# microsoft/ISLE

Measured on AMD Instinct MI355X. Metric: docs/sec end-to-end ISLETrain (SVD+k-means), k=1000; top-k σ rel-err, higher is better.
Workload: dtype f32

## Files before the change

include/isle_hip.h:

```cpp
#ifndef ISLE_HIP_H
#define ISLE_HIP_H

#include <stddef.h>
#include <stdint.h>

#ifdef __cplusplus
extern "C" {
#endif

typedef struct isle_ctx isle_ctx;

enum {
  ISLE_OK = 0,
  ISLE_E_ARG = -1,
  ISLE_E_HIP = -2,
  ISLE_E_NOCONV = -3,
  ISLE_E_NUMERIC = -4,
  ISLE_E_COMM = -5
};

isle_ctx* isle_hip_create(int device_id);
void isle_hip_destroy(isle_ctx* ctx);
const char* isle_hip_last_error(isle_ctx* ctx);

// ... 39 lines not shown
                   uint64_t* original_cols, float* zetas);
int isle_hip_shape(isle_ctx* ctx, uint64_t* vocab_size, uint64_t* num_docs, uint64_t* nnz,
                   uint64_t* doc_offset, uint64_t* docs_global);

int isle_hip_frobenius(isle_ctx* ctx, float* out);

int isle_hip_gram_apply(isle_ctx* ctx, const float* X_colmajor, int b, float* Z_colmajor);

int isle_hip_operator_form(isle_ctx* ctx, int* form);

int isle_hip_switch_info(int index, const char** name, const char** kind, const char** what);

int isle_hip_block_ks(isle_ctx* ctx, int nev, int ncv, int maxit, int blk, float tol, uint64_t seed,
                      float* evals, int* nconv, int* restarts, int* napplies);

int isle_hip_block_ks_dense(isle_ctx* ctx, const float* A_colmajor, uint64_t n, int nev, int ncv, int maxit, int blk,
                            float tol, uint64_t seed, const float* start_block, float* evals, float* U_colmajor,
                            int* nconv, int* nconv_ref_rule, int* restarts, int* napplies);

int isle_hip_get_U(isle_ctx* ctx, float* U_colmajor);
int isle_hip_set_U(isle_ctx* ctx, const float* U_colmajor, int k);

int isle_hip_eig_sym(isle_ctx* ctx, const float* S_colmajor, int n, float* evals_desc, float* vecs_colmajor);

int isle_hip_kmeanspp_projected(isle_ctx* ctx, int k, const uint64_t* inject_seeds, uint64_t rng_seed,
                                uint64_t* seeds_out, float* C_lowd, float* residual, int* rounds);

int isle_hip_host_rand(uint64_t seed, int n, uint32_t* out);

int isle_hip_get_min_dist(isle_ctx* ctx, float* min_dist);

int isle_hip_lloyds_projected(isle_ctx* ctx, int k, float* C_lowd, int max_reps, int* iters_run,
                              uint32_t* assign_out);

int isle_hip_lift_centers(isle_ctx* ctx, const float* in, int ld_in, int ncols, float* centers);

int isle_hip_lloyds_sparse(isle_ctx* ctx, int k, const float* centers_in, float* centers_out,
                           uint32_t* assign, int max_reps, int* iters_run);

int isle_hip_catchwords(isle_ctx* ctx, int num_topics, const uint32_t* assign, uint64_t r, double rho,
                        float* thresholds, int32_t* catch_topic, uint64_t* num_catchwords);

int isle_hip_topic_model(isle_ctx* ctx, int num_topics, uint64_t rank_threshold, float* model,
                         float* model_threshold, int32_t* top1, int32_t* top2, uint64_t* doc_topic_sums);
int isle_hip_get_doc_topic_sums(isle_ctx* ctx, int64_t* doc_offsets, uint32_t* topic, float* val);

int isle_hip_edge_topics(isle_ctx* ctx, const int64_t* pairs, int n, float primary_ratio, float* edge);

#define ISLE_EDGE_TABLE_MAX_TOPICS 8192
int isle_hip_select_edge_pairs(isle_ctx* ctx, const int32_t* top1, const int32_t* top2, uint64_t n_docs, int num_topics,
                               int64_t max_edge_topics, uint64_t min_docs, int64_t* pairs, uint64_t cap, uint64_t* n_selected,
                               uint64_t* n_candidates, uint64_t* threshold );

int isle_hip_topic_coherence(isle_ctx* ctx, int num_topics, int M, const uint32_t* top_words, double eps, double* coherence,
                             uint64_t* doc_freq, uint64_t* co_doc_freq);

int isle_hip_avg_topic_model(isle_ctx* ctx, int num_topics, float* model);

#define ISLE_MODEL_CATCH 0
#define ISLE_MODEL_AVG 1
#define ISLE_MODEL_HOST 2
#define ISLE_MODEL_LOADED 3

int isle_hip_model_top_words(isle_ctx* ctx, int which, const float* model_host, uint64_t vocab, int ncols, int n, uint32_t* ids, float* weights);

int isle_hip_edge_top_words(isle_ctx* ctx, int which, const float* model_host, uint64_t vocab, int ncols, const int64_t* pairs, int n_edge,
// ... 79 lines not shown
```

isle_amd/_lib.py:

```python
import ctypes as C
import os

_HERE = os.path.dirname(os.path.abspath(__file__))
_LIB = None

_P, _I, _U64, _F = C.c_void_p, C.c_int, C.c_uint64, C.c_float
SYMBOLS = {
    "isle_hip_create": (_P, [_I]),
    "isle_hip_destroy": (None, [_P]),
    "isle_hip_last_error": (C.c_char_p, [_P]),
    "isle_hip_switch_info": (_I, [_I, _P, _P, _P]),
    "isle_hip_comm_unique_id": (_I, [_P]),
    "isle_hip_comm_init": (_I, [_P, _I, _I, _P]),
    "isle_hip_comm_init_host": (_I, [_P, _I, _I, _P, _P]),
    "isle_hip_plan_shards": (_I, [_U64, _P, _I, _P]),
    "isle_hip_upload_csc_u64": (_I, [_P, _U64, _U64, _U64, _P, _P, _P, _U64, _U64]),
    "isle_hip_upload_csc_u32": (_I, [_P, _U64, _U64, _U64, _P, _P, _P, _U64, _U64]),
    "isle_hip_upload_counts_u32": (_I, [_P, _U64, _U64, _U64, _P, _P, _P, _U64, _U64]),
    "isle_hip_ingest_tdf": (_I, [_P, _P, _U64, _U64, _U64, _U64, _P, _P]),
    "isle_hip_feed_begin": (_I, [_P, _U64, _U64, _U64]),
    "isle_hip_feed_entries": (_I, [_P, _U64, _P, _P, _P]),
    "isle_hip_feed_entries_pieces": (_I, [_P, _U64, _P, _P, _P, _U64]),
    "isle_hip_feed_finalize": (_I, [_P, _U64, _U64, _P, _P]),
    "isle_hip_tdf_begin": (_I, [_P, _U64, _U64, _U64, _U64]),
# ... 14 lines not shown
    "isle_hip_topic_coherence": (_I, [_P, _I, _I, _P, C.c_double, _P, _P, _P]),
    "isle_hip_avg_topic_model": (_I, [_P, _I, _P]),
    "isle_hip_model_top_words": (_I, [_P, _I, _P, _U64, _I, _I, _P, _P]),
    "isle_hip_topic_diversity": (_I, [_P, _I, _I, _P, _P]),
    "isle_hip_model_text": (_I, [_P, _I, _P, _U64, _I, _I, _P, _P, _P, _P]),
    "isle_hip_edge_topics_text": (_I, [_P, _P, _I, _F, _I, _P, _P, _P, _P]),
    "isle_hip_entry_text": (_I, [_F, _I, _P]),
    "isle_hip_load_model_text": (_I, [_P, _P, _U64, _U64, _I, _I, C.c_uint, _P]),
    "isle_hip_get_loaded_model": (_I, [_P, _P, _P, _P]),
    "isle_hip_parse_weight": (_I, [_P, _U64, _I, _P]),
    "isle_hip_log_combinatorial": (_I, [_P, _P, _P]),
    "isle_hip_distinct_top_five": (_I, [_P, _I, _P, _P, _P, _P, _P, _P]),
    "isle_hip_top_five_count_rule": (_I, [_P, _U64, C.c_int32, _P]),
    "isle_hip_frobenius": (_I, [_P, _P]),
    "isle_hip_gram_apply": (_I, [_P, _P, _I, _P]),
    "isle_hip_operator_form": (_I, [_P, _P]),
    "isle_hip_infer": (_I, [_P, C.c_uint64, _I, _P, C.c_uint64, C.c_uint64, _P, _P, _P, _I, C.c_float, C.c_float, _P, _P, _P, _P, _P]),
    "isle_hip_infer_resident": (_I, [_P, _I, _P, _U64, _I, _U64, _U64, _I, _F, _F, _U64, _P, _P, _P, _P, _P]),
    "isle_hip_get_infer_entries": (_I, [_P, _P, _P, _P]),
    "isle_hip_infer_text": (_I, [_P, _I, _U64, _U64, _U64, _P, _P, _P, _P]),
    "isle_hip_doc_line_text": (_I, [_U64, _U64, _F, _P]),
    "isle_hip_doc_report_text": (_I, [_P, _I, _U64, _U64, _P, _P, _P, _P]),
    "isle_hip_top_two_line_text": (_I, [_U64, _U64, _U64, _P]),
    "isle_hip_avg_doc_sz": (_I, [_P, _P]),
    "isle_hip_block_ks": (_I, [_P, _I, _I, _I, _I, _F, _U64, _P, _P, _P, _P]),
    "isle_hip_block_ks_dense": (_I, [_P, _P, _U64, _I, _I, _I, _I, _F, _U64, _P, _P, _P, _P, _P, _P, _P]),
    "isle_hip_get_U": (_I, [_P, _P]),
    "isle_hip_set_U": (_I, [_P, _P, _I]),
    "isle_hip_eig_sym": (_I, [_P, _P, _I, _P, _P]),
    "isle_hip_kmeanspp_projected": (_I, [_P, _I, _P, _U64, _P, _P, _P, _P]),
    "isle_hip_get_min_dist": (_I, [_P, _P]),
    "isle_hip_host_rand": (_I, [_U64, _I, _P]),
    "isle_hip_lloyds_projected": (_I, [_P, _I, _P, _I, _P, _P]),
    "isle_hip_lift_centers": (_I, [_P, _P, _I, _I, _P]),
    "isle_hip_lloyds_sparse": (_I, [_P, _I, _P, _P, _P, _I, _P]),
    "isle_hip_timing_enable": (_I, [_P, _I]),
    "isle_hip_timing_reset": (_I, [_P]),
    "isle_hip_timing_get": (_I, [_P, _P, _P]),
    "isle_hip_synchronize": (_I, [_P]),
}


class IsleHipError(RuntimeError):
    pass


def library_path():
    return os.environ.get("ISLE_HIP_LIB") or os.path.join(_HERE, "libisle_hip.so")


def load_library():
    global _LIB
    if _LIB is not None:
        return _LIB
    path = library_path()
    if not os.path.exists(path):
        raise IsleHipError(
            "%s not found — build it with `make -C isle_amd/csrc` (or __graft_entry__.build()). "
            "There is no CPU fallback for the ISLE hot path." % path)
    lib = C.CDLL(path)
    for name, (res, args) in SYMBOLS.items():
        fn = getattr(lib, name)
        fn.restype = res
        fn.argtypes = args
    _LIB = lib
    return lib
# ... 1 lines not shown
```

isle_amd/csrc/api_kmeans.cpp:

```cpp
#include <algorithm>
#include <chrono>
#include <cmath>
#include <cstdarg>
#include <cstdlib>
#include <cstring>
#include <numeric>

#include "api_internal.h"

#ifndef ISLE_PROJ_FULL_NUM
#define ISLE_PROJ_FULL_NUM 1
#define ISLE_PROJ_FULL_DEN 3
#endif
static void choose_movers(const std::vector<float>& delta, int k, int group, int G, YyMovers* mv, std::vector<float>* gmax_excl,
                          const std::vector<uint32_t>* slot_of_id = nullptr ) {
  mv->n = 0;
  if ((int)delta.size() != k || k <= 16) return;
  std::vector<int> ord(k);
  std::iota(ord.begin(), ord.end(), 0);
  std::partial_sort(ord.begin(), ord.begin() + 11, ord.end(), [&](int a, int b) { return delta[a] > delta[b] || (delta[a] == delta[b] && a < b); });
  const float ref = delta[ord[10]];
  for (int j = 0; j < 10; ++j)
    if (delta[ord[j]] > 2.0f * ref && delta[ord[j]] > 1e-4f) mv->id[mv->n++] = (uint32_t)ord[j];
  if (!mv->n) return;
// ... 302 lines not shown
  bool from_kmpp;
  bool pt_sorted;
  bool delta_sums;
  bool movers;
};
struct ProjScalars {
  float* delta;
  HamTop* top;
  float* tmove;
};
}

static ProjPlan proj_plan(isle_ctx* c, int k, const float* C_lowd) {
  ProjPlan p;
  p.hamerly = !c->knob_on(KN_NO_HAMERLY) && (c->Pt_ready || c->Pt2_ready);
  p.T = (k + 31) / 32;
  p.TL = (p.T + 3) & ~3;
  p.tiles = p.hamerly && k > 224 && p.T <= 32 && !c->knob_is(KN_PROJ_BOUNDS, "hamerly");
  p.from_kmpp = p.tiles && c->kmpp_track_k == k && c->kmpp_P_gen == c->P_gen && c->P_ready && !c->knob_zero(KN_KMPP_TRACK) &&
                c->kmpp_C_host.size() == (size_t)k * k && memcmp(c->kmpp_C_host.data(), C_lowd, (size_t)k * k * sizeof(float)) == 0;
  p.pt_sorted = !c->knob_zero(KN_PT_SORT);
  p.delta_sums = !c->knob_is(KN_PROJ_SUMS, "fresh") && c->D < (1ull << 31);
  p.movers = !c->knob_zero(KN_YY_MOVERS) && c->D > 0;
  return p;
}

static int proj_reserve(isle_ctx* c, const ProjPlan& p, int k, ProjScalars* sc) {
  const uint64_t D = c->D;
  const int ldk = c->ldk;
  if (p.hamerly) {
    HIPCHK(c, c->hub.reserve(D ? D : 1));
    HIPCHK(c, c->hlb.reserve(D ? D : 1));
    HIPCHK(c, c->active.reserve(D + 1));
    HIPCHK(c, c->Pa.reserve((size_t)(D ? D : 1) * ldk));
    HIPCHK(c, c->pna.reserve(D ? D : 1));
    HIPCHK(c, c->Cold.reserve((size_t)k * ldk + k + 8));
  }
  if (p.tiles) {
    HIPCHK(c, c->ptlb.reserve((size_t)(D ? D : 1) * p.TL));
    HIPCHK(c, c->pneed.reserve(D ? D : 1));
    HIPCHK(c, c->pcand.reserve(D + 1));
    HIPCHK(c, c->small.reserve(4096));
  }
  if (p.delta_sums) HIPCHK(c, c->proj_counted.reserve(D ? D : 1));
  if (c->multi()) HIPCHK(c, c->Csum_local.reserve((size_t)k * ldk));
  sc->delta = p.hamerly ? c->Cold.p + (size_t)k * ldk : nullptr;
  sc->top = p.hamerly ? reinterpret_cast<HamTop*>(c->Cold.p + (size_t)k * ldk + round4(k)) : nullptr;
  sc->tmove = p.tiles ? c->small.p : nullptr;
  return 0;
}

static int proj_assign_first(isle_ctx* c, const ProjPlan& p, int k) {
  const uint64_t D = c->D;
  const int ldk = c->ldk;
  if (p.from_kmpp) return k_kmpp_to_tiles(c, D, k, c->pnorm.p, c->cnorm.p, c->kmpp_best.p, c->assign.p, c->hub.p, p.TL);
  if (p.tiles)
    return k_proj_assign_tiles(c, c->P.p, c->pnorm.p, D, k, ldk, c->Cdev.p, c->cnorm.p, c->assign.p, c->hub.p, c->ptlb.p, p.TL, nullptr, 0, nullptr, nullptr,
                               nullptr);
  return k_proj_assign(c, c->P.p, c->pnorm.p, D, k, ldk, c->Cdev.p, c->cnorm.p, c->assign.p, p.hamerly ? c->hub.p : nullptr,
                       p.hamerly ? c->hlb.p : nullptr);
}

static int debug_tile_stats(isle_ctx* c, int it, uint32_t na, int T) {
  const uint64_t D = c->D;
  std::vector<uint32_t> act(na), need(D);
  if (na) HIPCHK(c, hipMemcpy(act.data(), c->active.p, na * sizeof(uint32_t), hipMemcpyDeviceToHost));
  if (D) HIPCHK(c, hipMemcpy(need.data(), c->pneed.p, D * sizeof(uint32_t), hipMemcpyDeviceToHost));
// ... 109 lines not shown
  HIPCHK(c, hipStreamSynchronize(c->stream));
  isle_host_mark("lloyds_projected: centres uploaded");
  ProjScalars sc;
  ISLECHK(proj_reserve(c, plan, k, &sc));
  c->kmpp_track_k = 0;
  if (c->knob_on(KN_DEBUG_HAMERLY)) fprintf(stderr, "[projected Lloyd] first assignment %s\n", plan.from_kmpp ? "taken from the k-means++ rounds" : "computed");
  StopRule stop(c, k);
  int it = 0;
  std::vector<float> pdelta_host;
  isle_host_mark("lloyds_projected: loop starts");
  for (; it < max_reps; ++it) {
    ISLECHK(k_rownorms(c, c->Cdev.p, k, k, ldk, c->cnorm.p));
    if (it == 0 || !plan.hamerly) ISLECHK(proj_assign_first(c, plan, k));
    else if (plan.tiles) ISLECHK(proj_reassign_tiles(c, plan, sc, k, it, pdelta_host));
    else ISLECHK(proj_reassign_hamerly(c, sc, k, it));
    ISLECHK(k_count_sizes(c, c->assign.p, D, k, c->counts.p));
    std::vector<long long> sizes;
    ISLECHK(proj_update_centres(c, plan, k, it, sizes));
    if (plan.hamerly && it + 1 < max_reps) ISLECHK(proj_movements(c, plan, sc, k, pdelta_host));
    bool conv = false;
    ISLECHK(stop.converged(sizes, c->assign.p, &conv));
    if (conv) {
      ++it;
      break;
    }
  }
  isle_host_mark("lloyds_projected: loop done");
  HIPCHK(c, hipMemcpyAsync(Ch, c->Cdev.p, ch_bytes, hipMemcpyDeviceToHost, c->stream));
  if (assign_out && D) HIPCHK(c, hipMemcpyAsync(assign_out, c->assign.p, D * sizeof(uint32_t), hipMemcpyDeviceToHost, c->stream));
  HIPCHK(c, hipStreamSynchronize(c->stream));
  centres_unpack(C_lowd, Ch, k, ldk);
  if (iters_run) *iters_run = it;
  isle_host_mark("lloyds_projected: exit");
  return 0;
}

static int install_centers(isle_ctx* c, int ncols) {
  const int ld = round4(ncols);
  HIPCHK(c, c->centers_rm.reserve((size_t)c->V * ld));
  HIPCHK(c, hipMemsetAsync(c->centers_rm.p, 0, (size_t)c->V * ld * sizeof(float), c->stream));
  ISLECHK(k_transpose(c, c->centers_cm.p, c->V, ncols, c->V, c->centers_rm.p, ld));
  c->centers_ready = true;
  c->centers_k = ncols;
  return 0;
}

extern "C" int isle_hip_lift_centers(isle_ctx* c, const float* in, int ld_in, int ncols, float* centers) {
  if (!c || !in || ncols < 1) return ISLE_E_ARG;
  ISLECHK(isle_enter(c));
  if (c->U_k == 0 || ld_in < c->U_k) return isle_fail(c, ISLE_E_ARG, "lift: need U and ld_in >= k");
  isle_host_mark("lift: entry");
  HIPCHK(c, c->Csum.reserve((size_t)ld_in * ncols));
  {
    const size_t in_bytes = (size_t)ld_in * ncols * sizeof(float);
    HIPCHK(c, c->pin_stage.reserve(in_bytes));
    memcpy(c->pin_stage.p, in, in_bytes);
    HIPCHK(c, hipMemcpyAsync(c->Csum.p, c->pin_stage.p, in_bytes, hipMemcpyHostToDevice, c->stream));
  }
  HIPCHK(c, c->centers_cm.reserve((size_t)c->V * ncols));
  ISLECHK(k_gemm_nn(c, c->Ucm.p, c->V, c->U_k, c->Csum.p, ld_in, ncols, c->centers_cm.p, ISLE_T_LIFT));
  ISLECHK(install_centers(c, ncols));
  HIPCHK(c, c->lift_C.reserve((size_t)ld_in * ncols));
  HIPCHK(c, hipMemcpyAsync(c->lift_C.p, c->Csum.p, (size_t)ld_in * ncols * sizeof(float), hipMemcpyDeviceToDevice, c->stream));
  c->lift_ld = ld_in;
  c->lift_k = ncols;
  c->lift_valid = true;
// ... 326 lines not shown
```

isle_amd/csrc/common.h:

```cpp
#pragma once
#include <hip/hip_runtime.h>
#include <rccl/rccl.h>

#include <atomic>
#include <cstdint>
#include <cstdio>
#include <functional>
#include <string>
#include <thread>
#include <vector>

#include "gl_plan.h"

struct IsleLaunchRefused {
  const char* file = nullptr;
  int line = 0;
  unsigned long long threads = 0;
};
inline IsleLaunchRefused& isle_launch_refused() {
  static thread_local IsleLaunchRefused r;
  return r;
}
inline bool isle_launch_fits(dim3 g, dim3 b, const char* file, int line) {
  const unsigned long long blocks = (unsigned long long)g.x * g.y * g.z, threads = blocks * ((unsigned long long)b.x * b.y * b.z);
// ... 557 lines not shown
int k_load_model_text(isle_ctx* c, const unsigned char* text_dev, uint64_t n, uint64_t V, uint32_t ncols, int format, unsigned base, float* model_dev,
                      uint64_t* nentries, uint64_t* err_key);

int k_coherence_counts(isle_ctx* c, const std::vector<uint32_t>& U, const std::vector<uint32_t>& part_off, const std::vector<uint32_t>& part_hi,
                       std::vector<uint32_t>& counts, int* passes);

int k_avg_model(isle_ctx* c, uint32_t k);
int k_model_top_words(isle_ctx* c, const float* model_dev, uint64_t V, uint32_t ncols, int n, uint32_t* ids_dev, float* weights_dev);
int k_topic_diversity(isle_ctx* c, const float* model_dev, uint64_t V, uint32_t k, double* dist_dev, double* abar_dev, int32_t* finite_dev,
                      uint32_t* kprime);
int k_edge_top_words(isle_ctx* c, const float* model_dev, uint64_t V, const int64_t* pairs_dev, uint32_t n_edge, float a, float b, int n,
                     uint32_t* ids_dev, float* weights_dev);

int k_edge_select(isle_ctx* c, const int32_t* top1_dev, const int32_t* top2_dev, uint64_t D, uint32_t k, uint64_t max_edge_topics, uint64_t min_docs,
                  int64_t* pairs_host, uint64_t cap, uint64_t* n_selected, uint64_t* n_candidates, uint64_t* threshold, uint64_t* bad_doc);

int k_log_combinatorial(isle_ctx* c, float* out, uint64_t* max_words);
int k_top_five_runs(isle_ctx* c, uint64_t* n_out, std::vector<uint64_t>& runs, float* tuples);

int k_ensure_pt(isle_ctx* c);
int k_vtf(isle_ctx* c, const float* Vb, uint64_t n, int m, const float* F, int b, float* coef , uint64_t ld = 0);
int k_update(isle_ctx* c, float* F, uint64_t n, int b, const float* Vb, int m, const float* coef, uint64_t ld = 0);
int k_panel_qr(isle_ctx* c, float* F, uint64_t n, int w, float* Qdst, float* R_host , int* rank_out);
int k_panel_qr_kernels(isle_ctx* c, float* F, uint64_t n, int w, float* Qdst, int* meta_dev , float* Rout_dev );
int k_randu(isle_ctx* c, float* F, uint64_t count, uint64_t seed);
int k_gemm_nn(isle_ctx* c, const float* A, uint64_t M, int K, const float* B, int ldb, int N, float* C, int family = ISLE_T_ROTATE);
int k_gemm_nn_assign(isle_ctx* c, const float* A, uint64_t M, int K, const float* B, int ldb, int N, float* C, int family);
bool k_gemm_assign_fused_ok(isle_ctx* c, uint64_t M, int K, int N);
int k_gemm_assign_yy(isle_ctx* c, const float* A, const float* Arm, int lda_rm, const float* an, uint64_t M, int K, const float* B, int ldb, int N, int G,
                     const float* cn, const float* dn, const float* cn_max, uint32_t* assign, float* ub, float* lb, int family, const void* A2 = nullptr,
                     const uint32_t* map2 = nullptr );
int k_gemm_assign_tiles(isle_ctx* c, const float* A, const float* Arm, int lda_rm, uint64_t M, int K, const float* B, int ldb, int N, int TL, const float* cn,
                        const float* pn, const float* cmax, uint32_t* assign, float* ub, float* tlb, int family, const uint32_t* map0 = nullptr,
                        const void* A2 = nullptr, const uint32_t* map2 = nullptr);
int k_gemm_split_a(isle_ctx* c, const float* A, uint64_t M, int K, void* A2);
size_t k_gemm_split_a_bytes(uint64_t M, int K);
int k_transpose(isle_ctx* c, const float* in, uint64_t rows, uint64_t cols, uint64_t ld_in, float* out, uint64_t ld_out);
int k_jacobi_eig(isle_ctx* c, const float* S_host, int n, float* evals_host, float* vecs_dev );
int k_eig_small(isle_ctx* c, const float* S_host, int n, float* evals_host, float* vecs_dev , int nvec);
int k_colnorms_rm(isle_ctx* c, const float* Mrm, uint64_t rows, int k, int ldk, float* out, const float* Sub = nullptr);
int k_scale_centers(isle_ctx* c, float* Crm, uint64_t rows, int k, int ldk, const int* counts);

int k_tridiag_eig(isle_ctx* c, const float* S_host, int n, float* evals_host, float* vecs_dev, int nvec);

int k_member_lists(isle_ctx* c, const uint32_t* assign, uint64_t D, int k, const int* counts_dev, int* max_out, std::vector<int>* counts_host = nullptr);
int k_member_lists_dev(isle_ctx* c, const uint32_t* assign, uint64_t D, int k, const int* counts_dev);
int k_yy_delta(isle_ctx* c, float* delta_dev, int k, int G, int group, float* gmax_dev, const uint32_t* id_of_slot = nullptr);
int k_max_f32(isle_ctx* c, const float* v, int n, float* out_dev);
int k_compact_rows(isle_ctx* c, const float* P, const float* pn, int ldk, const uint32_t* active, uint32_t n, float* Pa, float* pna);
int k_kmpp_update(isle_ctx* c, const float* P, const float* pn, uint64_t D, int k, int ldk, const float* newC, int nc, float* min_dist, int s_old = -1,
                  bool track = false);
int k_kmpp_to_tiles(isle_ctx* c, uint64_t D, int k, const float* pn, const float* cn, const float* best, uint32_t* assign, float* ub, int TL);
int k_scan_f2d(isle_ctx* c, const float* in, uint64_t n, double* cum );
int k_search(isle_ctx* c, const double* cum, uint64_t n, const double* dice_dev, int nd, uint64_t* out_dev);
int k_search_args(isle_ctx* c, const double* cum, uint64_t n, const double* dice_host, int nd , uint64_t* out_dev);
int k_fetch_rows(isle_ctx* c, const float* P, int ldk, const uint64_t* local_ids , int n, float* dst);
int k_pack2(isle_ctx* c, const double* a, const float* b , double* out2);
int k_search_frac(isle_ctx* c, const double* cum, uint64_t n, const float* last , const double* frac_host, int nd ,
                  uint64_t* out_dev );
int k_proj_assign(isle_ctx* c, const float* P, const float* pn, uint64_t D, int k, int ldk, const float* C, const float* cn, uint32_t* assign,
                  float* ub = nullptr, float* lb = nullptr);
int k_proj_assign_active(isle_ctx* c, const float* P, const float* pn, int k, int ldk, const float* C, const float* cn,
                         const uint32_t* active, uint32_t n, float* Pa, float* pna, uint32_t* assign, float* ub, float* lb);
bool k_proj_full_by_gemm(isle_ctx* c, uint64_t D, int k);
int k_proj_assign_tiles(isle_ctx* c, const float* P, const float* pn, uint64_t D, int k, int ldk, const float* C, const float* cn, uint32_t* assign,
                        float* ub, float* tlb, int TL, const uint32_t* active, uint32_t n, const uint32_t* need, float* Pa, float* pna);
int k_rownorms_diff(isle_ctx* c, const float* A, const float* B, int rows, int k, int ldk, float* out);
int k_rownorms(isle_ctx* c, const float* M, int rows, int k, int ldk, float* out);
int k_proj_accumulate(isle_ctx* c, const float* P, uint64_t D, int k, int ldk, const uint32_t* assign, float* Csum, int* counts);
// ... 7 lines not shown
```

isle_amd/csrc/dense.hip:

```cpp
#include <algorithm>
#include <cstdlib>

#include "gemm_f32.h"
#include "gemm_bf16x3.h"

#include "common.h"
#include "gridbar.h"
#include "hamerly.h"

typedef float floatx16 __attribute__((ext_vector_type(16)));

constexpr int VTF_CG = 32;
constexpr int vtf_rc(int BT) { return BT <= 12 ? 1024 : (BT <= 16 ? 512 : 256); }

template <int BT>
__global__ __launch_bounds__(256) void vtf_partial_k(const float* __restrict__ Vb, uint64_t n, uint64_t ld, int m, const float* __restrict__ F,
                                                      int b, double* __restrict__ part ) {
  constexpr int VTF_RC = vtf_rc(BT);
  __shared__ float Fs[BT][VTF_RC];
  const uint64_t r0 = (uint64_t)blockIdx.x * VTF_RC;
  const int rc = (int)min((uint64_t)VTF_RC, n - r0);
  for (int idx = threadIdx.x; idx < BT * VTF_RC; idx += 256) {
    const int j = idx / VTF_RC, r = idx - j * VTF_RC;
    Fs[j][r] = (j < b && r < rc) ? F[(uint64_t)j * ld + r0 + r] : 0.f;
// ... 781 lines not shown
                                                       uint32_t* __restrict__ redo, uint32_t* __restrict__ nredo) {
  const uint32_t i = blockIdx.x * 256 + threadIdx.x;
  const bool in = i < n;
  bool open = false;
  if (in) {
    const uint32_t d = map ? map[i] : i;
    const AssignPick p = assign_pick(part, i, nslot);
    const float nd = pn[d];
    const float eps = eta * (nd + *cmax_p);
    assign[d] = p.bidx;
    float uu, ll, l2;
    hamerly_store_bounds(p.best + eps, fmaxf(p.m2 - eps, 0.f), nd + p.ax, &uu, &l2);
    hamerly_store_bounds(p.best + eps, p.best + eps, nd + *cmax_p, &uu, &ll);
    ub[d] = uu;
    lb[(size_t)d * TL + (p.bidx >> 5)] = l2;
    open = eta > 0.f && p.run2 - p.best <= 2.f * eps;
  }
  if (eta > 0.f) {
    const uint32_t at = block_append_slot(open, nredo);
    if (open) redo[at] = map ? map[i] : i;
  }
}
bool k_gemm_assign_fused_ok(isle_ctx* c, uint64_t M, int K, int N) {
  return !c->knob_zero(KN_GEMM_BF16X3) && !c->knob_zero(KN_GEMM_EPILOGUE) && N >= 64 && K >= 32 && (M + 255) / 256 * (uint64_t)((N + 255) / 256) >= 512 &&
         M < (1ull << 32);
}
using Gemm2Huge = isle_gemm3::Cfg<2, 2, 4, 4, 4, 16, 2>;
using Gemm2Dma = isle_gemm3::CfgDma<2, 16>;
int k_gemm_split_a(isle_ctx* c, const float* A, uint64_t M, int K, void* A2) {
  HIPCHK(c, isle_gemm3::split_a(c->stream, A, M, K, A2, Gemm2Dma::TK));
  return 0;
}
size_t k_gemm_split_a_bytes(uint64_t M, int K) { return isle_gemm3::a2_units(M, K, Gemm2Dma::TK) * 16; }
template <class MakeEpi, class Combine>
static int gemm_assign_two_pass(isle_ctx* c, const float* A, const float* Arm, int lda_rm, const float* rown, uint64_t M, int K, const float* B, int ldb, int N,
                                MakeEpi make, Combine combine, const uint32_t* map0 = nullptr ,
                                const void* A2 = nullptr ,
                                const uint32_t* map2 = nullptr ) {
  auto need_a = [&]() -> int {
    if (A) return 0;
    ISLECHK(k_ensure_pt(c));
    A = c->Pt.p;
    return 0;
  };
  const int nslot = (N + 63) / 64;
  static_assert(sizeof(AssignRec) == 20, "");
  const char* gt = c->knob(KN_GEMM_TERMS);
  const bool two = !(gt && atoi(gt) == 3) && Arm != nullptr;
  HIPCHK(c, c->gemm_b3.reserve((size_t)3 * isle_gemm3::kp8_of(K) * isle_gemm3::np_of<Gemm3Huge>(N)));
  HIPCHK(c, c->assign_part.reserve((size_t)M * nslot * 5));
  AssignRec* part = reinterpret_cast<AssignRec*>(c->assign_part.p);
  if (!two) {
    ISLECHK(need_a());
    HIPCHK(c, isle_gemm3::launch<Gemm3Huge>(c->stream, A, M, K, B, ldb, N, c->gemm_b3.p, make(part, map0, 0.f)));
    combine(part, (uint32_t)M, map0, 0.f, nullptr, nullptr);
    HIPCHK(c, hipGetLastError());
    return 0;
  }
  const float eta2 = ga_eta(K);
  HIPCHK(c, c->ga_redo.reserve(M + 1));
  uint32_t* nredo = c->ga_redo.p + M;
  HIPCHK(c, hipMemsetAsync(nredo, 0, sizeof(uint32_t), c->stream));
  if (A2 && !c->knob_zero(KN_GEMM_DMA)) {
    HIPCHK(c, isle_gemm3::launch_dma<Gemm2Dma>(c->stream, A2, M, K, B, ldb, N, c->gemm_b3.p, make(part, map2 ? map2 : map0, eta2)));
    combine(part, (uint32_t)M, map2 ? map2 : map0, eta2, c->ga_redo.p, nredo);
  } else {
    ISLECHK(need_a());
    HIPCHK(c, isle_gemm3::launch<Gemm2Huge>(c->stream, A, M, K, B, ldb, N, c->gemm_b3.p, make(part, map0, eta2)));
    combine(part, (uint32_t)M, map0, eta2, c->ga_redo.p, nredo);
  }
  HIPCHK(c, hipGetLastError());
  uint32_t n = 0;
  ISLECHK(isle_fetch_u32(c, nredo, &c->pin_small()->redo_count, &n));
// ... 7 lines not shown
    HIPCHK(c, hipGetLastError());
    return 0;
  }
  HIPCHK(c, c->ga_rows.reserve((size_t)n * lda_rm));
  HIPCHK(c, c->ga_rown.reserve(n));
  ISLECHK(k_compact_rows(c, Arm, rown, lda_rm, c->ga_redo.p, n, c->ga_rows.p, c->ga_rown.p));
  HIPCHK(c, isle_gemm3::launch<Gemm3Huge>(c->stream, c->ga_rows.p, (uint64_t)n, K, B, ldb, N, c->gemm_b3.p, make(part, c->ga_redo.p, 0.f)));
  combine(part, n, c->ga_redo.p, 0.f, nullptr, nullptr);
  HIPCHK(c, hipGetLastError());
  return 0;
}
int k_gemm_assign_yy(isle_ctx* c, const float* A, const float* Arm, int lda_rm, const float* an, uint64_t M, int K, const float* B, int ldb, int N, int G,
                     const float* cn, const float* dn, const float* cn_max, uint32_t* assign, float* ub, float* lb, int family, const void* A2,
                     const uint32_t* map2) {
  TimeScope ts(c, family);
  const int nslot = (N + 63) / 64;
  HIPCHK(c, c->ga_bn.reserve((size_t)N + 4));
  float* bmax = c->ga_bn.p + N;
  if (an) {
    ISLECHK(k_rownorms(c, B, N, K, ldb, c->ga_bn.p));
    ISLECHK(k_max_f32(c, c->ga_bn.p, N, bmax));
  }
  return gemm_assign_two_pass(
      c, A, an ? Arm : nullptr, lda_rm, an, M, K, B, ldb, N,
      [&](AssignRec* part, const uint32_t* map, float eta) { return YyGroupEpi{cn, dn, cn_max, lb, G, nslot, part, map, eta, an, bmax}; },
      [&](const AssignRec* part, uint32_t n, const uint32_t* map, float eta, uint32_t* redo, uint32_t* nredo) {
        hipLaunchKernelGGL(yy_first_combine_k, dim3(cdiv(n, 256)), dim3(256), 0, c->stream, part, nslot, n, G, dn, cn_max, assign, ub, lb, map, eta, an, bmax, redo,
                           nredo);
      },
      nullptr, A2, map2);
}
int k_gemm_assign_tiles(isle_ctx* c, const float* A, const float* Arm, int lda_rm, uint64_t M, int K, const float* B, int ldb, int N, int TL, const float* cn,
                        const float* pn, const float* cmax, uint32_t* assign, float* ub, float* tlb, int family, const uint32_t* map0, const void* A2,
                        const uint32_t* map2) {
  TimeScope ts(c, family);
  const int nslot = (N + 63) / 64;
  return gemm_assign_two_pass(
      c, A, Arm, lda_rm, pn, M, K, B, ldb, N,
      [&](AssignRec* part, const uint32_t* map, float eta) { return TileEpi{cn, pn, cmax, tlb, TL, nslot, part, map, eta}; },
      [&](const AssignRec* part, uint32_t n, const uint32_t* map, float eta, uint32_t* redo, uint32_t* nredo) {
        hipLaunchKernelGGL(tiles_combine_k, dim3(cdiv(n, 256)), dim3(256), 0, c->stream, part, nslot, n, TL, pn, cmax, assign, ub, tlb, map, eta, redo, nredo);
      },
      map0, A2, map2);
}

__global__ __launch_bounds__(256) void transpose_k(const float* __restrict__ in, uint64_t rows, uint64_t cols, uint64_t ld_in,
                                                    float* __restrict__ out, uint64_t ld_out) {
  __shared__ float t[32][33];
  const uint64_t r0 = (uint64_t)blockIdx.x * 32, c0 = (uint64_t)blockIdx.y * 32;
  const int tx = threadIdx.x & 31, ty = threadIdx.x >> 5;
  for (int yy = ty; yy < 32; yy += 8) {
    const uint64_t r = r0 + tx, cc = c0 + yy;
    t[yy][tx] = (r < rows && cc < cols) ? in[cc * ld_in + r] : 0.f;
  }
  __syncthreads();
  for (int yy = ty; yy < 32; yy += 8) {
    const uint64_t r = r0 + yy, cc = c0 + tx;
    if (r < rows && cc < cols) out[r * ld_out + cc] = t[tx][yy];
  }
}
int k_transpose(isle_ctx* c, const float* in, uint64_t rows, uint64_t cols, uint64_t ld_in, float* out, uint64_t ld_out) {
  if (rows == 0 || cols == 0) return 0;
  const uint64_t cb = cdiv(cols, 32);
  const uint64_t rows_per = std::max<uint64_t>(32, ((1ull << 31) / 256 / cb) * 32);
  for (uint64_t r0 = 0; r0 < rows; r0 += rows_per) {
    const uint64_t nr = std::min(rows_per, rows - r0);
    dim3 g((unsigned)cdiv(nr, 32), (unsigned)cb), blk(256);
    hipLaunchKernelGGL(transpose_k, g, blk, 0, c->stream, in + r0, nr, cols, ld_in, out + r0 * ld_out, ld_out);
    HIPCHK(c, hipGetLastError());
  }
  return 0;
}

int k_ensure_pt(isle_ctx* c) {
  if (c->Pt_ready) return 0;
  if (!c->P_ready || !c->D) return isle_fail(c, ISLE_E_ARG, "no projection to transpose");
// ... 423 lines not shown
```

isle_amd/csrc/gemm_bf16x3.h:

```cpp
#pragma once
#include <hip/hip_runtime.h>
#include <stdint.h>

namespace isle_gemm3 {

typedef __bf16 bf16x8 __attribute__((ext_vector_type(8)));
typedef __bf16 bf16x4 __attribute__((ext_vector_type(4)));
typedef float f32x16 __attribute__((ext_vector_type(16)));

__device__ inline void split3(float x, __bf16& x0, __bf16& x1, __bf16& x2) {
  x0 = (__bf16)x;
  const float r1 = x - (float)x0;
  x1 = (__bf16)r1;
  const float r2 = r1 - (float)x1;
  x2 = (__bf16)r2;
}

__global__ __launch_bounds__(256) void gemm3_split_b_k(const float* __restrict__ B, int ldb, int K, int N, int Kp8, int Np, bf16x8* __restrict__ B3) {
  const size_t i = (size_t)blockIdx.x * 256 + threadIdx.x;
  if (i >= (size_t)Kp8 * Np) return;
  const int q = (int)(i / Np), n = (int)(i - (size_t)q * Np);
  bf16x8 v[3];
#pragma unroll
  for (int j = 0; j < 8; ++j) {
// ... 291 lines not shown
  static constexpr int NS = NS_;
  static constexpr int WMT = 2, WNT = 2, WAVES_M = 4, WAVES_N = 4, TK = TK_, KO = TK_ / 8, NP = 2, OCC = 4;
  static constexpr int TM = 256, TN = 256, NT = 1024;
  static constexpr int A_STAGE = NP * KO * TM, B_STAGE = NP * KO * TN, STAGE = A_STAGE + B_STAGE;
  static constexpr int PPW = STAGE / 64 / 16;
  static constexpr size_t LDS_BYTES = (size_t)NS * STAGE * 16;
  static_assert(TK_ == 16 || TK_ == 32, "slabs of 16 or 32");
};
inline int nslab_of(int K, int TK) { return (K + TK - 1) / TK; }
inline size_t a2_units(uint64_t M, int K, int TK = 16) { return (size_t)((M + 255) / 256) * nslab_of(K, TK) * (4 * (TK / 8)) * 256; }

__global__ __launch_bounds__(256) void gemm2_split_a_k(const float* __restrict__ A, uint64_t M, int K, int nslab, int KO, bf16x8* __restrict__ A2) {
  const uint64_t mb = blockIdx.x, m = mb * 256 + threadIdx.x;
  const int q = blockIdx.y;
  bf16x8 v0, v1;
#pragma unroll
  for (int j = 0; j < 8; ++j) {
    const int k = 8 * q + j;
    const float x = (m < M && k < K) ? A[(uint64_t)k * M + m] : 0.f;
    const __bf16 x0 = (__bf16)x;
    v0[j] = x0;
    v1[j] = (__bf16)(x - (float)x0);
  }
  const size_t base = ((mb * nslab + (size_t)(q / KO)) * (2 * KO) + (size_t)(q % KO)) * 256 + threadIdx.x;
  A2[base] = v0;
  A2[base + (size_t)KO * 256] = v1;
}
inline hipError_t split_a(hipStream_t stream, const float* A, uint64_t M, int K, void* A2, int TK = 16) {
  const int nslab = nslab_of(K, TK);
  const uint64_t nMB = (M + 255) / 256;
  if (nMB == 0) return hipSuccess;
  if (nMB >= (1ull << 31)) return hipErrorInvalidValue;
  hipLaunchKernelGGL(gemm2_split_a_k, dim3((uint32_t)nMB, (uint32_t)(nslab * (TK / 8))), dim3(256), 0, stream, A, M, K, nslab, TK / 8, reinterpret_cast<bf16x8*>(A2));
  return hipGetLastError();
}

template <class CF, class Epi>
__global__ __launch_bounds__(CF::NT) void gemm_bf16x2_dma_k(const bf16x8* __restrict__ A2, uint64_t M, int K, const bf16x8* __restrict__ B3, int Kp8, int Np,
                                                             int N, uint32_t nMB, uint32_t nNT, Epi epi) {
  constexpr int TM = CF::TM, TN = CF::TN, WMT = CF::WMT, WNT = CF::WNT, KO = CF::KO, NP = CF::NP, NS = CF::NS, TK = CF::TK, PPW = CF::PPW;
  static_assert((NS & (NS - 1)) == 0 && NS >= 2 && NS <= 4, "ring of 2 or 4 stages");
  extern __shared__ bf16x8 ldsr[];
  const uint32_t wg = blockIdx.x, xcd = wg & 7u, slot = wg >> 3;
  const uint32_t mb = (slot / nNT) * 8u + xcd, nt = slot % nNT;
  if (mb >= nMB) return;
  const uint64_t m0 = (uint64_t)mb * TM;
  const int n0 = (int)nt * TN;
  const int tid = threadIdx.x, lane = tid & 63;
  const int wave = __builtin_amdgcn_readfirstlane(tid >> 6);
  const int l31 = lane & 31, h = lane >> 5;
  const int wm = wave % CF::WAVES_M, wn = wave / CF::WAVES_M;
  const int nslab = (K + TK - 1) / TK;
  const bool mine_a = wave < 8;
  const int w8 = mine_a ? wave : wave - 8;
  const bf16x8* ga = A2 + ((size_t)mb * nslab) * CF::A_STAGE + (size_t)(w8 * PPW) * 64 + lane;
  const bf16x8* gb[PPW];
#pragma unroll
  for (int i = 0; i < PPW; ++i) {
    const int u = (w8 * PPW + i) * 64 + lane;
    gb[i] = B3 + ((size_t)((u / (KO * 256)) * Kp8 + ((u >> 8) % KO))) * Np + n0 + (u & 255);
  }
  const uint32_t lpiece = (uint32_t)(((mine_a ? 0 : CF::A_STAGE) + w8 * PPW * 64) * 16);
  auto issue = [&](int s) {
    char* l = reinterpret_cast<char*>(ldsr) + (size_t)(s & (NS - 1)) * CF::STAGE * 16 + lpiece;
    if (mine_a) {
      const bf16x8* g = ga + (size_t)s * CF::A_STAGE;
// ... 78 lines not shown
```

isle_amd/csrc/kmeans.hip:

```cpp
#include <algorithm>
#include <cstdlib>
#include <vector>

#include <cstring>

#include "common.h"
#include "hamerly.h"
#include "scan.h"

typedef float floatx16 __attribute__((ext_vector_type(16)));
constexpr int CS_ITEMS = 16;
enum { PR_ARGMIN = 0, PR_MINDIST = 1, PR_TILES = 2 };
template <int MODE>
static int launch_proj_reg(isle_ctx* c, uint64_t D, int k, int ldk, const float* C, const float* cn, const float* pn, uint32_t* assign,
                           float* min_dist, bool* done, const float* Pt = nullptr, const uint32_t* map = nullptr, float* ub = nullptr,
                           float* lb = nullptr, const uint32_t* need = nullptr, int TL = 0);

template <int NIT>
__global__ __launch_bounds__(256) void kmpp_update_k(const float* __restrict__ P, const float* __restrict__ pn, uint32_t D, int ldk,
                                                      const float* __restrict__ newC, const float* __restrict__ cn, int nc,
                                                      float* __restrict__ min_dist) {
  const int lane = threadIdx.x & 63;
  const uint32_t d = blockIdx.x * 4 + (threadIdx.x >> 6);
  if (d >= D) return;
// ... 919 lines not shown
}

bool k_proj_full_by_gemm(isle_ctx* c, uint64_t D, int k) {
  const char* pf = c->knob(KN_PROJ_FULL);
  return (c->Pt_ready || c->Pt2_ready) && D > 0 && k >= 64 && (k_gemm_assign_fused_ok(c, D, k, k) || isle_scratch_ok(c, c->dotsT.cap, (double)D * k * sizeof(float))) &&
         ((2.0 * (double)D * k * k >= 2e10 && !(pf && !strcmp(pf, "fused"))) || (pf && !strcmp(pf, "gemm")));
}
int k_proj_assign_tiles(isle_ctx* c, const float* P, const float* pn, uint64_t D, int k, int ldk, const float* C, const float* cn, uint32_t* assign,
                        float* ub, float* tlb, int TL, const uint32_t* active, uint32_t n, const uint32_t* need, float* Pa, float* pna) {
  TimeScope ts(c, ISLE_T_LLOYD_PROJ);
  bool done = false;
  if (!active) {
    if (k_proj_full_by_gemm(c, D, k)) {
      if (k_gemm_assign_fused_ok(c, D, k, k)) {
        HIPCHK(c, c->cmax_buf.reserve(4));
        ISLECHK(k_max_f32(c, cn, k, c->cmax_buf.p));
        const bool a2 = c->Pt2_ready && P == c->P.p;
        return k_gemm_assign_tiles(c, c->Pt_ready ? c->Pt.p : nullptr, P, ldk, D, k, C, ldk, k, TL, cn, pn, c->cmax_buf.p, assign, ub, tlb, ISLE_T_LLOYD_PROJ, nullptr,
                                   a2 ? c->Pt2.p : nullptr, a2 && c->Pt2_pos ? c->dperm.p : nullptr);
      }
      HIPCHK(c, c->dotsT.reserve((size_t)D * k));
      ISLECHK(k_ensure_pt(c));
      ISLECHK(k_gemm_nn_assign(c, c->Pt.p, D, k, C, ldk, k, c->dotsT.p, ISLE_T_LLOYD_PROJ));
      hipLaunchKernelGGL(proj_dots_tiles_k, dim3(cdiv(D, 256)), dim3(256), 0, c->stream, c->dotsT.p, (uint32_t)D, k, pn, cn, assign, ub, tlb, TL);
      HIPCHK(c, hipGetLastError());
      return 0;
    }
    ISLECHK(launch_proj_reg<PR_TILES>(c, D, k, ldk, C, cn, pn, assign, nullptr, &done, nullptr, nullptr, ub, tlb, nullptr, TL));
  } else {
    if (n == 0) return 0;
    {
      const char* pa = c->knob(KN_PROJ_ACTIVE);
      const bool by_gemm = pa ? !strcmp(pa, "gemm") : true;
      if (by_gemm && k_gemm_assign_fused_ok(c, n, k, k)) {
        ISLECHK(k_compact_rows(c, P, pn, ldk, active, n, Pa, pna));
        HIPCHK(c, c->cmax_buf.reserve(4));
        ISLECHK(k_max_f32(c, cn, k, c->cmax_buf.p));
        return k_gemm_assign_tiles(c, Pa, P, ldk, n, k, C, ldk, k, TL, cn, pn, c->cmax_buf.p, assign, ub, tlb, ISLE_T_LLOYD_PROJ, active);
      }
    }
    if (need && n > 256 && !c->knob_zero(KN_PT_SORT)) {
      HIPCHK(c, c->gl_key_a.reserve(n));
      HIPCHK(c, c->gl_key_b.reserve(n));
      HIPCHK(c, c->gl_val_a.reserve(n));
      HIPCHK(c, c->gl_val_b.reserve(n));
      hipLaunchKernelGGL(pt_need_keys_k, dim3(cdiv(n, 256)), dim3(256), 0, c->stream, active, n, need, c->gl_key_a.p, c->gl_val_a.p);
      HIPCHK(c, hipGetLastError());
      bool in_a = true;
      ISLECHK(k_sort_pairs_u64(c, c->gl_key_a.p, c->gl_val_a.p, c->gl_key_b.p, c->gl_val_b.p, n, ((k + 31) / 32 + 7) & ~7, &in_a));
      active = in_a ? c->gl_val_a.p : c->gl_val_b.p;
    }
    ISLECHK(k_compact_rows(c, P, pn, ldk, active, n, Pa, pna));
    ISLECHK(launch_proj_reg<PR_TILES>(c, n, k, ldk, C, cn, pna, assign, nullptr, &done, Pa, active, ub, tlb, need, TL));
  }
  if (!done) return isle_fail(c, ISLE_E_ARG, "projected assignment with tile bounds: shape not covered (k = %d)", k);
  return 0;
}

int k_proj_assign(isle_ctx* c, const float* P, const float* pn, uint64_t D, int k, int ldk, const float* C, const float* cn,
                  uint32_t* assign, float* ub, float* lb) {
  {
    TimeScope ts(c, ISLE_T_LLOYD_PROJ);
    bool done = false;
    ISLECHK(launch_proj_reg<PR_ARGMIN>(c, D, k, ldk, C, cn, pn, assign, nullptr, &done, nullptr, nullptr, ub, lb));
    if (done) return 0;
  }
// ... 464 lines not shown
```

isle_amd/hot_path.py:

```python
import ctypes as C

import numpy as np

from ._lib import IsleHipError, load_library

TIMING_FAMILIES = ["gram_pass1", "gram_pass2", "ortho", "qr", "evd", "rotate", "project", "kmpp", "lloyd_proj",
                   "sparse_assign", "sparse_update", "op_build", "comm", "threshold", "post", "ingest", "infer", "lift"]

BLOCK_KS_MAX_ITERS = 100
BLOCK_KS_BLOCK_SIZE = 10
BLOCK_KS_TOLERANCE = 1e-4
MAX_KMEANS_LOWD_REPS = 10
MAX_KMEANS_REPS = 10


W0_C, EPS2_C, EPS3_C, RHO_C = 1.0, 1.0 / 3.0, 5.0, 1.1


def catchword_rank(num_docs, num_topics, sample_rate=None):
    x = EPS2_C * W0_C * float(np.float32(num_docs))
    if sample_rate is not None:
        x = x * float(np.float32(sample_rate))
    return int(np.floor(x / float(np.float32(2.0 * num_topics))))

# ... 589 lines not shown
    def set_U(self, U):
        U = np.asfortranarray(U, dtype=np.float32)
        self._chk(self._lib.isle_hip_set_U(self._h, _p(U), U.shape[1]))

    def eig_sym(self, S):
        S = np.asfortranarray(S, dtype=np.float32)
        n = S.shape[0]
        e = np.empty(n, np.float32)
        v = np.empty((n, n), np.float32, order="F")
        self._chk(self._lib.isle_hip_eig_sym(self._h, _p(S), n, _p(e), _p(v)))
        return e, v

    def kmeans_init_on_projected_space(self, k, inject_seeds=None, rng_seed=1):
        seeds = np.empty(k, np.uint64)
        Cl = np.empty((k, k), np.float32)
        res, rounds = C.c_float(), C.c_int()
        inj = None if inject_seeds is None else np.ascontiguousarray(inject_seeds, np.uint64)
        self._chk(self._lib.isle_hip_kmeanspp_projected(self._h, k, _p(inj), rng_seed, _p(seeds), _p(Cl), C.byref(res),
                                                       C.byref(rounds)))
        return dict(seeds=seeds, C_lowd=Cl, residual=res.value, rounds=rounds.value)

    def get_min_dist(self):
        md = np.empty(self.D, np.float32)
        self._chk(self._lib.isle_hip_get_min_dist(self._h, _p(md)))
        return md

    def run_lloyds_on_projected_space(self, k, C_lowd, max_reps=MAX_KMEANS_LOWD_REPS):
        Cl = np.array(C_lowd, dtype=np.float32, order="C", copy=True)
        it = C.c_int()
        assign = np.empty(self.D, np.uint32)
        self._chk(self._lib.isle_hip_lloyds_projected(self._h, k, _p(Cl), max_reps, C.byref(it), _p(assign)))
        return dict(C_lowd=Cl, iters=it.value, assign=assign)

    def left_multiply_by_U(self, C_lowd, fetch=True):
        Cl = np.ascontiguousarray(C_lowd, dtype=np.float32)
        n, k = Cl.shape
        out = np.empty((self.V, n), np.float32, order="F") if fetch else None
        self._chk(self._lib.isle_hip_lift_centers(self._h, _p(Cl), k, n, _p(out)))
        return out

    def run_lloyds(self, k, centers=None, max_reps=MAX_KMEANS_REPS, fetch_centers=True):
        cin = None if centers is None else np.asfortranarray(centers, dtype=np.float32)
        cout = np.empty((self.V, k), np.float32, order="F") if fetch_centers else None
        assign = np.empty(self.D, np.uint32)
        it = C.c_int()
        self._chk(self._lib.isle_hip_lloyds_sparse(self._h, k, _p(cin), _p(cout), _p(assign), max_reps, C.byref(it)))
        return dict(centers=cout, assign=assign, iters=it.value)

    def infer(self, model_by_word, offs, rows, counts, iters=15, Lf=10.0, avg_doc_sz=None, want_weights=True):
        M = np.ascontiguousarray(model_by_word, np.float32)
        V, k = M.shape
        offs = np.ascontiguousarray(offs, np.int64)
        rows = np.ascontiguousarray(rows, np.uint32)
        counts = np.ascontiguousarray(counts, np.float32)
        D = offs.shape[0] - 1
        if avg_doc_sz is None:
            nz = int((np.diff(offs) > 0).sum())
            avg_doc_sz = float(int(counts.astype(np.float64).sum()) // max(nz, 1))
        W = np.empty((D, k), np.float32) if want_weights else None
        tt = np.empty((D, 5), np.int32)
        tw = np.empty((D, 5), np.float32)
        llh = np.empty((D, 2), np.float32)
        nc = C.c_uint64()
        self._chk(self._lib.isle_hip_infer(self._h, V, k, _p(M), D, rows.shape[0], _p(counts), _p(rows), _p(offs), int(iters), float(Lf),
                                           float(avg_doc_sz), _p(W) if want_weights else None, _p(tt), _p(tw), _p(llh), C.byref(nc)))
        return dict(weights=W, top_topic=tt, top_weight=tw, llh=llh, nconverged=int(nc.value), avg_doc_sz=avg_doc_sz)
# ... 87 lines not shown
```

Baseline: 4.759 million.

## Fuse active-row gather with bf16 split-image build in projected Lloyd assignment

```diff
diff --git a/include/isle_hip.h b/include/isle_hip.h
--- a/include/isle_hip.h
+++ b/include/isle_hip.h
@@ -95,6 +95,9 @@
 
 int isle_hip_lloyds_projected(isle_ctx* ctx, int k, float* C_lowd, int max_reps, int* iters_run,
                               uint32_t* assign_out);
+
+int isle_hip_gather_split_image(isle_ctx* ctx, int k, const uint32_t* docs, uint32_t n, int fused, void* image, uint64_t image_bytes,
+                                float* norms);
 
 int isle_hip_lift_centers(isle_ctx* ctx, const float* in, int ld_in, int ncols, float* centers);
 
diff --git a/isle_amd/_lib.py b/isle_amd/_lib.py
--- a/isle_amd/_lib.py
+++ b/isle_amd/_lib.py
@@ -70,6 +70,7 @@
     "isle_hip_get_min_dist": (_I, [_P, _P]),
     "isle_hip_host_rand": (_I, [_U64, _I, _P]),
     "isle_hip_lloyds_projected": (_I, [_P, _I, _P, _I, _P, _P]),
+    "isle_hip_gather_split_image": (_I, [_P, _I, _P, C.c_uint32, _I, _P, _U64, _P]),
     "isle_hip_lift_centers": (_I, [_P, _P, _I, _I, _P]),
     "isle_hip_lloyds_sparse": (_I, [_P, _I, _P, _P, _P, _I, _P]),
     "isle_hip_timing_enable": (_I, [_P, _I]),
diff --git a/isle_amd/csrc/api_kmeans.cpp b/isle_amd/csrc/api_kmeans.cpp
--- a/isle_amd/csrc/api_kmeans.cpp
+++ b/isle_amd/csrc/api_kmeans.cpp
@@ -358,7 +358,7 @@
     HIPCHK(c, c->hub.reserve(D ? D : 1));
     HIPCHK(c, c->hlb.reserve(D ? D : 1));
     HIPCHK(c, c->active.reserve(D + 1));
-    HIPCHK(c, c->Pa.reserve((size_t)(D ? D : 1) * ldk));
+    HIPCHK(c, c->Pa.reserve(std::max((size_t)(D ? D : 1) * ldk, k_gemm_image_bytes(D, k) / sizeof(float))));
     HIPCHK(c, c->pna.reserve(D ? D : 1));
     HIPCHK(c, c->Cold.reserve((size_t)k * ldk + k + 8));
   }
@@ -534,6 +534,35 @@
   centres_unpack(C_lowd, Ch, k, ldk);
   if (iters_run) *iters_run = it;
   isle_host_mark("lloyds_projected: exit");
+  return 0;
+}
+
+extern "C" int isle_hip_gather_split_image(isle_ctx* c, int k, const uint32_t* docs, uint32_t n, int fused, void* image, uint64_t image_bytes,
+                                           float* norms) {
+  if (!c || !docs || !image || k < 1 || n == 0) return ISLE_E_ARG;
+  ISLECHK(isle_enter(c));
+  ISLECHK(ensure_P(c, k));
+  const uint64_t D = c->D;
+  const int ldk = c->ldk;
+  if (n > D) return isle_fail(c, ISLE_E_ARG, "gather_split_image: %u rows of %llu", n, (unsigned long long)D);
+  for (uint32_t i = 0; i < n; ++i)
+    if (docs[i] >= D) return isle_fail(c, ISLE_E_ARG, "gather_split_image: document %u of %llu", docs[i], (unsigned long long)D);
+  const size_t bytes = k_gemm_image_bytes(n, k);
+  if (image_bytes != bytes) return isle_fail(c, ISLE_E_ARG, "gather_split_image: the image takes %zu bytes", bytes);
+  HIPCHK(c, c->active.reserve(D + 1));
+  HIPCHK(c, c->pna.reserve(D));
+  HIPCHK(c, c->Pa.reserve(std::max((size_t)D * ldk, k_gemm_image_bytes(D, k) / sizeof(float))));
+  HIPCHK(c, hipMemcpyAsync(c->active.p, docs, (size_t)n * sizeof(uint32_t), hipMemcpyHostToDevice, c->stream));
+  if (fused) {
+    ISLECHK(k_gemm_gather_split_a(c, c->P.p, ldk, c->active.p, n, k, c->Pa.p, c->pnorm.p, c->pna.p));
+  } else {
+    HIPCHK(c, c->ga_rows.reserve((size_t)n * ldk));
+    ISLECHK(k_compact_rows(c, c->P.p, c->pnorm.p, ldk, c->active.p, n, c->ga_rows.p, c->pna.p));
+    ISLECHK(k_gemm_split_a(c, c->ga_rows.p, n, k, c->Pa.p));
+  }
+  HIPCHK(c, hipMemcpyAsync(image, c->Pa.p, bytes, hipMemcpyDeviceToHost, c->stream));
+  if (norms) HIPCHK(c, hipMemcpyAsync(norms, c->pna.p, (size_t)n * sizeof(float), hipMemcpyDeviceToHost, c->stream));
+  HIPCHK(c, hipStreamSynchronize(c->stream));
   return 0;
 }
 
diff --git a/isle_amd/csrc/common.h b/isle_amd/csrc/common.h
--- a/isle_amd/csrc/common.h
+++ b/isle_amd/csrc/common.h
@@ -613,9 +613,13 @@
                      const uint32_t* map2 = nullptr );
 int k_gemm_assign_tiles(isle_ctx* c, const float* A, const float* Arm, int lda_rm, uint64_t M, int K, const float* B, int ldb, int N, int TL, const float* cn,
                         const float* pn, const float* cmax, uint32_t* assign, float* ub, float* tlb, int family, const uint32_t* map0 = nullptr,
-                        const void* A2 = nullptr, const uint32_t* map2 = nullptr);
+                        const void* A2 = nullptr, const uint32_t* map2 = nullptr,
+                        float* gather_a = nullptr ,
+                        float* gather_an = nullptr );
 int k_gemm_split_a(isle_ctx* c, const float* A, uint64_t M, int K, void* A2);
 size_t k_gemm_split_a_bytes(uint64_t M, int K);
+int k_gemm_gather_split_a(isle_ctx* c, const float* P, int ldp, const uint32_t* list, uint32_t n, int K, void* A2, const float* pn, float* pna);
+size_t k_gemm_image_bytes(uint64_t M, int K);
 int k_transpose(isle_ctx* c, const float* in, uint64_t rows, uint64_t cols, uint64_t ld_in, float* out, uint64_t ld_out);
 int k_jacobi_eig(isle_ctx* c, const float* S_host, int n, float* evals_host, float* vecs_dev );
 int k_eig_small(isle_ctx* c, const float* S_host, int n, float* evals_host, float* vecs_dev , int nvec);
diff --git a/isle_amd/csrc/dense.hip b/isle_amd/csrc/dense.hip
--- a/isle_amd/csrc/dense.hip
+++ b/isle_amd/csrc/dense.hip
@@ -837,13 +837,25 @@
   return 0;
 }
 size_t k_gemm_split_a_bytes(uint64_t M, int K) { return isle_gemm3::a2_units(M, K, Gemm2Dma::TK) * 16; }
+int k_gemm_gather_split_a(isle_ctx* c, const float* P, int ldp, const uint32_t* list, uint32_t n, int K, void* A2, const float* pn, float* pna) {
+  HIPCHK(c, isle_gemm3::gather_split_a(c->stream, P, ldp, list, n, K, A2, pn, pna, Gemm2Dma::TK));
+  return 0;
+}
+size_t k_gemm_image_bytes(uint64_t M, int K) { return (size_t)((M + 255) / 256) * isle_gemm3::nslab_of(K, Gemm2Dma::TK) * Gemm2Dma::A_STAGE * 16; }
 template <class MakeEpi, class Combine>
 static int gemm_assign_two_pass(isle_ctx* c, const float* A, const float* Arm, int lda_rm, const float* rown, uint64_t M, int K, const float* B, int ldb, int N,
                                 MakeEpi make, Combine combine, const uint32_t* map0 = nullptr ,
                                 const void* A2 = nullptr ,
-                                const uint32_t* map2 = nullptr ) {
+                                const uint32_t* map2 = nullptr ,
+                                float* gather_a = nullptr ,
+                                float* gather_an = nullptr ) {
   auto need_a = [&]() -> int {
     if (A) return 0;
+    if (gather_a) {
+      ISLECHK(k_compact_rows(c, Arm, rown, lda_rm, map0, (uint32_t)M, gather_a, gather_an));
+      A = gather_a;
+      return 0;
+    }
     ISLECHK(k_ensure_pt(c));
     A = c->Pt.p;
     return 0;
@@ -917,16 +929,17 @@
 }
 int k_gemm_assign_tiles(isle_ctx* c, const float* A, const float* Arm, int lda_rm, uint64_t M, int K, const float* B, int ldb, int N, int TL, const float* cn,
                         const float* pn, const float* cmax, uint32_t* assign, float* ub, float* tlb, int family, const uint32_t* map0, const void* A2,
-                        const uint32_t* map2) {
+                        const uint32_t* map2, float* gather_a, float* gather_an) {
   TimeScope ts(c, family);
   const int nslot = (N + 63) / 64;
+  if (gather_a && (A || !Arm || !map0 || map2 != map0 || !gather_an)) return isle_fail(c, ISLE_E_ARG, "assignment product: a gathered operand is its image, its list and P");
   return gemm_assign_two_pass(
       c, A, Arm, lda_rm, pn, M, K, B, ldb, N,
       [&](AssignRec* part, const uint32_t* map, float eta) { return TileEpi{cn, pn, cmax, tlb, TL, nslot, part, map, eta}; },
       [&](const AssignRec* part, uint32_t n, const uint32_t* map, float eta, uint32_t* redo, uint32_t* nredo) {
         hipLaunchKernelGGL(tiles_combine_k, dim3(cdiv(n, 256)), dim3(256), 0, c->stream, part, nslot, n, TL, pn, cmax, assign, ub, tlb, map, eta, redo, nredo);
       },
-      map0, A2, map2);
+      map0, A2, map2, gather_a, gather_an);
 }
 
 __global__ __launch_bounds__(256) void transpose_k(const float* __restrict__ in, uint64_t rows, uint64_t cols, uint64_t ld_in,
diff --git a/isle_amd/csrc/gemm_bf16x3.h b/isle_amd/csrc/gemm_bf16x3.h
--- a/isle_amd/csrc/gemm_bf16x3.h
+++ b/isle_amd/csrc/gemm_bf16x3.h
@@ -347,6 +347,82 @@
   if (nMB == 0) return hipSuccess;
   if (nMB >= (1ull << 31)) return hipErrorInvalidValue;
   hipLaunchKernelGGL(gemm2_split_a_k, dim3((uint32_t)nMB, (uint32_t)(nslab * (TK / 8))), dim3(256), 0, stream, A, M, K, nslab, TK / 8, reinterpret_cast<bf16x8*>(A2));
+  return hipGetLastError();
+}
+
+constexpr int GS_ROWS = 64, GS_LD = 65;
+constexpr size_t GS_LDS_BYTES = (size_t)64 * GS_LD * 16;
+__global__ __launch_bounds__(256) void gemm2_gather_split_a_k(const float* __restrict__ P, int ldp, const uint32_t* __restrict__ list, uint32_t n, int K,
+                                                               int nslab, int KO, bf16x8* __restrict__ A2, const float* __restrict__ pn,
+                                                               float* __restrict__ pna) {
+  extern __shared__ uint4 gs[];
+  const uint32_t i0 = blockIdx.x * GS_ROWS;
+  const size_t mb = blockIdx.x >> 2;
+  const uint32_t r0 = (blockIdx.x & 3u) * GS_ROWS;
+  const int lane = threadIdx.x & 63, w = threadIdx.x >> 6;
+  const bool any = i0 < n;
+  const bool mine = i0 + (uint32_t)lane < n;
+  const uint32_t myd = any ? list[min(i0 + (uint32_t)lane, n - 1)] : 0u;
+  const int nq = nslab * KO;
+  for (int q0 = 0; q0 < nq; q0 += 32) {
+    __syncthreads();
+    if (any) {
+      const int j = 8 * q0 + 4 * lane;
+      float4 v[16];
+#pragma unroll
+      for (int u = 0; u < 16; ++u) {
+        const uint32_t d = (uint32_t)__shfl((int)myd, w * 16 + u);
+        v[u] = *reinterpret_cast<const float4*>(P + (size_t)d * ldp + min(j, ldp - 4));
+      }
+#pragma unroll
+      for (int u = 0; u < 16; ++u) {
+        const float x[4] = {j + 0 < K ? v[u].x : 0.f, j + 1 < K ? v[u].y : 0.f, j + 2 < K ? v[u].z : 0.f, j + 3 < K ? v[u].w : 0.f};
+        bf16x4 t0, t1;
+#pragma unroll
+        for (int t = 0; t < 4; ++t) {
+          const __bf16 x0 = (__bf16)x[t];
+          t0[t] = x0;
+          t1[t] = (__bf16)(x[t] - (float)x0);
+        }
+        const uint2 a0 = __builtin_bit_cast(uint2, t0), a1 = __builtin_bit_cast(uint2, t1);
+        const bool odd = lane & 1;
+        const uint2 send = odd ? a0 : a1;
+        uint2 recv;
+        recv.x = (uint32_t)__shfl_xor((int)send.x, 1);
+        recv.y = (uint32_t)__shfl_xor((int)send.y, 1);
+        const uint4 unit = odd ? make_uint4(recv.x, recv.y, a1.x, a1.y) : make_uint4(a0.x, a0.y, recv.x, recv.y);
+        gs[lane * GS_LD + w * 16 + u] = unit;
+      }
+    }
+    __syncthreads();
+#pragma unroll 4
+    for (int rr = 0; rr < 16; ++rr) {
+      const int run = w * 16 + rr, q = q0 + (run >> 1), term = run & 1;
+      if (q < nq) {
+        const uint4 unit = mine ? gs[run * GS_LD + lane] : make_uint4(0u, 0u, 0u, 0u);
+        const size_t at = ((mb * nslab + (size_t)(q / KO)) * (2 * KO) + (size_t)(term * KO + q % KO)) * 256 + r0 + lane;
+        reinterpret_cast<uint4*>(A2)[at] = unit;
+      }
+    }
+  }
+  if (pna && threadIdx.x < 64 && mine) pna[i0 + threadIdx.x] = pn[myd];
+}
+inline hipError_t gather_split_a(hipStream_t stream, const float* P, int ldp, const uint32_t* list, uint32_t n, int K, void* A2, const float* pn, float* pna,
+                                 int TK = 16) {
+  if (n == 0) return hipSuccess;
+  if (ldp < 4 || ldp % 4 != 0 || K > ldp) return hipErrorInvalidValue;
+  const uint32_t nMB = (n + 255u) / 256u;
+  static bool lds_attr_set[64] = {};
+  int dev = 0;
+  hipError_t e = hipGetDevice(&dev);
+  if (e != hipSuccess) return e;
+  if (dev < 0 || dev >= 64 || !lds_attr_set[dev]) {
+    e = hipFuncSetAttribute(reinterpret_cast<const void*>(&gemm2_gather_split_a_k), hipFuncAttributeMaxDynamicSharedMemorySize, (int)GS_LDS_BYTES);
+    if (e != hipSuccess) return e;
+    if (dev >= 0 && dev < 64) lds_attr_set[dev] = true;
+  }
+  hipLaunchKernelGGL(gemm2_gather_split_a_k, dim3(4 * nMB), dim3(256), GS_LDS_BYTES, stream, P, ldp, list, n, K, nslab_of(K, TK), TK / 8,
+                     reinterpret_cast<bf16x8*>(A2), pn, pna);
   return hipGetLastError();
 }
 
diff --git a/isle_amd/csrc/kmeans.hip b/isle_amd/csrc/kmeans.hip
--- a/isle_amd/csrc/kmeans.hip
+++ b/isle_amd/csrc/kmeans.hip
@@ -975,6 +975,17 @@
     {
       const char* pa = c->knob(KN_PROJ_ACTIVE);
       const bool by_gemm = pa ? !strcmp(pa, "gemm") : true;
+      const char* gt = c->knob(KN_GEMM_TERMS);
+      if (by_gemm && k_gemm_assign_fused_ok(c, n, k, k) && !c->knob_zero(KN_GEMM_DMA) && !(gt && atoi(gt) == 3) && ldk % 4 == 0) {
+        const size_t room = (Pa == c->Pa.p ? c->Pa.cap : (size_t)D * ldk) * sizeof(float);
+        if (k_gemm_image_bytes(n, k) > room)
+          return isle_fail(c, ISLE_E_ARG, "projected assignment: the split image of %u rows (%zu bytes) does not fit the gather buffer (%zu)", n,
+                           k_gemm_image_bytes(n, k), room);
+        ISLECHK(k_gemm_gather_split_a(c, P, ldk, active, n, k, Pa, nullptr, nullptr));
+        HIPCHK(c, c->cmax_buf.reserve(4));
+        ISLECHK(k_max_f32(c, cn, k, c->cmax_buf.p));
+        return k_gemm_assign_tiles(c, nullptr, P, ldk, n, k, C, ldk, k, TL, cn, pn, c->cmax_buf.p, assign, ub, tlb, ISLE_T_LLOYD_PROJ, active, Pa, active, Pa, pna);
+      }
       if (by_gemm && k_gemm_assign_fused_ok(c, n, k, k)) {
         ISLECHK(k_compact_rows(c, P, pn, ldk, active, n, Pa, pna));
         HIPCHK(c, c->cmax_buf.reserve(4));
diff --git a/isle_amd/hot_path.py b/isle_amd/hot_path.py
--- a/isle_amd/hot_path.py
+++ b/isle_amd/hot_path.py
@@ -645,6 +645,14 @@
         self._chk(self._lib.isle_hip_lloyds_projected(self._h, k, _p(Cl), max_reps, C.byref(it), _p(assign)))
         return dict(C_lowd=Cl, iters=it.value, assign=assign)
 
+    def gather_split_image(self, k, docs, fused=True):
+        docs = np.ascontiguousarray(docs, np.uint32)
+        n = docs.size
+        image = np.empty(-(-n // 256) * -(-k // 16) * 16384, np.uint8)
+        norms = np.empty(n, np.float32)
+        self._chk(self._lib.isle_hip_gather_split_image(self._h, k, _p(docs), n, 1 if fused else 0, _p(image), image.size, _p(norms)))
+        return image, norms
+
     def left_multiply_by_U(self, C_lowd, fetch=True):
         Cl = np.ascontiguousarray(C_lowd, dtype=np.float32)
         n, k = Cl.shape
```

Result: no change. 4.795 million (median of 6 runs) (+0.8%).
